# NathanBWaters/playaid_core

Hardware: AMD Instinct MI355X
Metric: 1080p frames/sec end-to-end (higher is better)
Workload: dtype f32; 1 GPU; configs[1]: 64 x 1080x1920 BGR frames per GPU per clip; parallelism=single GPU, lanes=2, ingest=raw BGR frames resident in HBM

## Files before the change

include/playaid_hip.h:

```cpp
#ifndef PLAYAID_HIP_H
#define PLAYAID_HIP_H

#include <stddef.h>
#include <stdint.h>

#ifdef __cplusplus
extern "C" {
#endif

#define PA_ABI_VERSION 15
#define PA_WEIGHT_MAGIC 0x31574150
#define PA_LSTM_MAGIC 0x314c4150
#define PA_ENCODER_MAGIC 0x31454150
#define PA_FEATURE_STRIDE 1024
#define PA_CROP 128

typedef enum pa_status {
    PA_OK = 0,
    PA_ERR_INVALID_ARG = -1,
    PA_ERR_HIP = -2,
    PA_ERR_BAD_WEIGHTS = -3,
    PA_ERR_CAPACITY = -4,
    PA_ERR_NO_DEVICE = -5,
    PA_ERR_NOT_READY = -6,
// ... 316 lines not shown
int pa_wino_conv3x3_splitk(const float* x, const float* ug, const float* bias, const float* residual, float* out, int32_t n,
                           int32_t height, int32_t width, int32_t cin, int32_t cout, int32_t bn, int32_t in_px_stride, int32_t out_px_stride,
                           int32_t out_pad, int32_t act, int32_t res_after, float* slab, size_t slab_floats, int32_t* tickets,
                           int32_t n_tickets, void* stream);

size_t pa_conv_weight_bytes(int32_t cin, int32_t cout, int32_t ksize, int32_t compute_dtype, int32_t has_residual);
int pa_conv_pack_weights(const float* w_host, int32_t cin, int32_t cout, int32_t ksize, int32_t compute_dtype, int32_t has_residual,
                         void* out_host);
int pa_conv2d(const float* x, const void* w, const float* bias, const float* residual, float* out, int32_t n, int32_t height,
              int32_t width, int32_t cin, int32_t cout, int32_t ksize, int32_t stride, int32_t in_pad, int32_t in_px_stride,
              int32_t out_px_stride, int32_t out_pad, int32_t act, int32_t res_after, int32_t compute_dtype, void* stream);
int pa_conv2d_branch(const float* x, const void* w, const float* bias, const float* residual, float* out, const float* w2, float* out2,
                     int32_t n, int32_t height, int32_t width, int32_t cin, int32_t cout, int32_t ksize, int32_t stride, int32_t in_pad,
                     int32_t in_px_stride, int32_t out_px_stride, int32_t out_pad, int32_t act, int32_t res_after, int32_t compute_dtype,
                     void* stream);

typedef struct pa_encoder pa_encoder;
size_t pa_encoder_blob_bytes(int32_t in_dim, int32_t hidden_dim, int32_t slots, int32_t enc_dim, int32_t num_layers,
                             int32_t ff_dim, int32_t num_actions);
int pa_encoder_create(int32_t device, int32_t in_dim, int32_t hidden_dim, int32_t slots, int32_t enc_dim, int32_t num_heads,
                      int32_t num_layers, int32_t ff_dim, int32_t num_actions, int32_t max_rows, const void* blob_host,
                      size_t blob_bytes, pa_encoder** out);
void pa_encoder_destroy(pa_encoder* h);
const char* pa_encoder_last_error(const pa_encoder* h);
int pa_encoder_forward(pa_encoder* h, const float* feats, int32_t ld, int32_t seq_len, int32_t batch, float* logp, void* stream);


int pa_profile_enable(pa_engine* e, int32_t on);
int pa_profile_read(pa_engine* e, pa_kernel_stat* stats, int32_t max_stats, int32_t* n_stats);

// ... 48 lines not shown
```

playaid_core_amd/_lib.py:

```python
from __future__ import annotations

import ctypes as C
import os

HERE = os.path.dirname(os.path.abspath(__file__))
LIB_PATH = os.environ.get("PA_LIB_PATH") or os.path.join(HERE, "libplayaid_hip.so")

PA_ABI_VERSION = 15
PA_DTYPE_F32 = 0
PA_DTYPE_BF16 = 1
PA_DTYPE_EMULATED_F32 = 2
DTYPES = {"f32": PA_DTYPE_F32, "bf16": PA_DTYPE_BF16, "emulated_f32": PA_DTYPE_EMULATED_F32}
PA_WEIGHT_MAGIC = 0x31574150
PA_LSTM_MAGIC = 0x314C4150
PA_ENCODER_MAGIC = 0x31454150
PA_FEATURE_STRIDE = 1024
PA_TRACE_STAGES = 20
DET_FORMS = ("not_run", "stem_direct", "stem_bf16", "wino", "patch", "pgemm", "pgemm_up", "psgemm", "psgemm_up", "igemm", "sppf",
             "maxpool", "upsample", "absorbed", "decode", "bgemm", "bgemm_up")
CN_FORMS = ("not_run", "stem_pool", "avgpool", "wino", "patch", "igemm_128x128", "igemm_128x64", "igemm_64x64", "psgemm",
            "bgemm", "bgemm_splitk", "avgpool_bf16")
LSTM_FORMS = ("not_run", "steps", "u1", "u2", "u4", "u8", "mfma")

PA_OK = 0
# ... 167 lines not shown
    ("pa_convnet_forward", C.c_int, [_P, _P, C.c_int32, _P, C.c_int32, _P]),
    ("pa_convnet_trace", C.c_int, [_P, _P, C.c_int32, C.c_int32, C.c_int32, _P, C.c_size_t, _P]),
    ("pa_convnet_layer_forms", C.c_int, [_P, _P, C.c_int32]),
    ("pa_detector_plan", C.c_int, [_P] * 5 + [C.c_int32] + [_P] * 7),
    ("pa_detector_plan_desc", C.c_int, [_P, _P, _P, C.c_int32, C.c_int32, C.c_longlong, _P, C.c_int32, C.c_longlong, _P]),
    ("pa_square_crops_src", C.c_int, [_P, _P, C.c_int32, C.c_int32, C.c_int32, _P, _P, C.c_int32, C.c_int32, C.c_int32, _P, _P, _P]),
    ("pa_wino_weight_floats", C.c_size_t, [C.c_int32, C.c_int32]),
    ("pa_wino_channels_per_workgroup", C.c_int, [C.c_int32, C.c_int64]),
    ("pa_wino_transform_weights", C.c_int, [_P, C.c_int32, C.c_int32, C.c_int32, _P]),
    ("pa_wino_conv3x3", C.c_int, [_P, _P, _P, _P, _P] + [C.c_int32] * 11 + [_P]),
    ("pa_conv_weight_bytes", C.c_size_t, [C.c_int32] * 5),
    ("pa_conv_pack_weights", C.c_int, [_P] + [C.c_int32] * 5 + [_P]),
    ("pa_conv2d", C.c_int, [_P, _P, _P, _P, _P] + [C.c_int32] * 14 + [_P]),
    ("pa_conv2d_branch", C.c_int, [_P, _P, _P, _P, _P, _P, _P] + [C.c_int32] * 14 + [_P]),
    ("pa_wino_conv3x3_splitk", C.c_int, [_P, _P, _P, _P, _P] + [C.c_int32] * 11 + [_P, C.c_size_t, _P, C.c_int32, _P]),
    ("pa_crop_resize_width", C.c_int, [_P, _P, C.c_int32, C.c_int32, C.c_int32, C.POINTER(C.c_int32), C.c_int32, C.c_int32, _P, C.c_int32,
                                       C.POINTER(C.c_int32), _P]),
    ("pa_encoder_blob_bytes", C.c_size_t, [C.c_int32] * 7),
    ("pa_encoder_create", C.c_int, [C.c_int32] * 10 + [_P, C.c_size_t, C.POINTER(_P)]),
    ("pa_encoder_destroy", None, [_P]),
    ("pa_encoder_last_error", C.c_char_p, [_P]),
    ("pa_encoder_forward", C.c_int, [_P, _P, C.c_int32, C.c_int32, C.c_int32, _P, _P]),
    ("pa_mjpeg_create", C.c_int, [C.c_int32, C.c_int32, C.c_int32, C.c_int32, C.c_size_t, C.POINTER(_P)]),
    ("pa_mjpeg_destroy", None, [_P]),
    ("pa_mjpeg_last_error", C.c_char_p, [_P]),
    ("pa_mjpeg_probe", C.c_int, [_P, C.c_size_t, C.POINTER(C.c_int32), C.c_char_p, C.c_size_t]),
    ("pa_mjpeg_set_sync_rounds", C.c_int, [_P, C.c_int32]),
    ("pa_mjpeg_set_groups", C.c_int, [_P, C.c_int32]),
    ("pa_mjpeg_last_sync_rounds", C.c_int, [_P]),
    ("pa_mjpeg_debug_counters", C.c_int, [_P]),
# ... 55 lines not shown
```

playaid_core_amd/conv.py:

```python
from __future__ import annotations

import ctypes as C

import numpy as np
import torch

from . import _lib


def pack_weights(w_oihw: np.ndarray, compute_dtype: str = "emulated_f32", has_residual: bool = False) -> np.ndarray:
    lib = _lib.load()
    w = np.ascontiguousarray(np.asarray(w_oihw, dtype=np.float32).transpose(0, 2, 3, 1))
    cout, k, _, cin = w.shape
    dt = _lib.DTYPES[compute_dtype]
    nbytes = lib.pa_conv_weight_bytes(cin, cout, k, dt, int(has_residual))
    if nbytes == 0:
        raise ValueError("cin and cout must be multiples of 32, the kernel 1x1 or 3x3, the dtype 'f32' or 'emulated_f32'")
    out = np.empty(nbytes, dtype=np.uint8)
    rc = lib.pa_conv_pack_weights(w.ctypes.data_as(C.c_void_p), cin, cout, k, dt, int(has_residual), out.ctypes.data_as(C.c_void_p))
    if rc:
        raise ValueError(f"pa_conv_pack_weights: status {rc}")
    return out


# ... 27 lines not shown
    n, hp, wp, cs = x_pad.shape
    h, wd = hp - 2 * in_pad, wp - 2 * in_pad
    oh, ow = h // stride, wd // stride
    mk = lambda: torch.zeros((n, oh + 2 * out_pad, ow + 2 * out_pad, cout), dtype=torch.float32, device=x_pad.device)
    out = mk() if out is None else out
    out2 = mk() if out2 is None else out2
    if out2.shape != out.shape:
        raise ValueError("out2 is addressed like out: same shape")
    ptr = lambda t_: C.c_void_p(t_.data_ptr()) if t_ is not None else C.c_void_p(0)
    stream = C.c_void_p(torch.cuda.current_stream(x_pad.device).cuda_stream)
    rc = lib.pa_conv2d_branch(ptr(x_pad), ptr(w), ptr(bias), C.c_void_p(0), ptr(out), ptr(w2), ptr(out2), n, h, wd, cin, cout, ksize, stride, in_pad, cs,
                              out.shape[3], out_pad, int(act), 0, _lib.DTYPES[compute_dtype], stream)
    if rc:
        raise ValueError(f"pa_conv2d_branch: status {rc}")
    return out, out2
```

playaid_core_amd/csrc/conv_rows.hip:

```cpp
#include "conv_rows.h"
#include "../../include/playaid_hip.h"

namespace pa {

GemmParams conv_row_params(const ConvRow& r) {
    const int oh = r.in_h / r.stride, ow = r.in_w / r.stride;
    const int in_hb = r.in_h + 2 * r.in_pad, in_wb = r.in_w + 2 * r.in_pad;
    const int out_hb = oh + 2 * r.out_pad, out_wb = ow + 2 * r.out_pad;
    GemmParams p;
    memset(&p, 0, sizeof(p));
    p.M = r.images * oh * ow;
    p.N = r.cout;
    p.taps = r.ksize * r.ksize;
    p.kw_taps = r.ksize;
    p.chunk = r.cin;
    p.ktot = p.taps * p.chunk;
    p.howo = oh * ow;
    p.wo = ow;
    p.in_px_stride = r.in_px_stride;
    p.in_row_stride = in_wb * r.in_px_stride;
    p.in_img_stride = in_hb * in_wb * r.in_px_stride;
    p.stride = r.stride;
    p.off_y = p.off_x = r.in_pad - (r.ksize - 1) / 2;
    p.out_px_stride = r.out_px_stride;
// ... 145 lines not shown
    const int oh = height / 2, ow = width / 2;
    const int in_wb = width + 2 * in_pad, in_hb = height + 2 * in_pad, out_wb = ow + 2 * out_pad, out_hb = oh + 2 * out_pad;
    if ((long long)n * in_hb * in_wb * in_px_stride >= (1ll << 29) || (long long)n * out_hb * out_wb * out_px_stride >= (1ll << 29)) return PA_ERR_CAPACITY;
    pa::GemmParams p = pa::conv_row_params({ n,  height, width, in_pad, in_px_stride,  cin, cout, 3, 2,
                                             out_pad, out_px_stride,  act, 0});
    p.act = x;
    p.wgt = static_cast<const float*>(w);
    p.bias = bias;
    p.out = out;
    p.wgt2 = w2;
    p.out2 = out2;
    const hipError_t e = pa::launch_pgemm(p, 64, static_cast<hipStream_t>(stream));
    return e == hipSuccess ? PA_OK : (e == hipErrorInvalidValue ? PA_ERR_INVALID_ARG : PA_ERR_HIP);
}

}
```

playaid_core_amd/csrc/igemm.hip:

```cpp
#include "tile_common.h"
#include <cstdio>
#include <cstdlib>

namespace pa {

#ifndef PA_COUNTED_VMCNT
#define PA_COUNTED_VMCNT 0
#endif

template <int BM, int BN, int BK, bool GATHER, int ABL = 0, bool SKIPW = false>
__global__ __launch_bounds__(256) void igemm_f32_kernel(const GemmParams p) {
    constexpr int MI = BM / 64;
    constexpr int NI = BN / 64;
    using Stage = Im2colStage<4, BK, BM, BN, GATHER>;
    constexpr int LDS_STRIDE = BK;
    constexpr int A_ROWS = Stage::A_ROWS, B_ROWS = Stage::B_ROWS;
    constexpr int STAGE = (BM + BN) * LDS_STRIDE;
    __shared__ __attribute__((aligned(16))) float lds[3 * STAGE];

    Stage st;
    st.setup(p);
    const int tile_m = st.tile_m, tile_n = st.tile_n, z = st.z;
    const int ks_begin = st.ks_begin, ks_end = st.ks_end;
    const int tid = threadIdx.x;
    const int wave_id = __builtin_amdgcn_readfirstlane(tid >> 6);
#define PA_ISSUE_STAGE(BUF)                                                \
    {                                                                      \
        float* As_w = lds + (BUF) * STAGE + wave_id * 256;                 \
        st.issue(p, As_w, As_w + BM * LDS_STRIDE);                         \
    }

    const int lane = tid & 63;
    const int wave = tid >> 6;
    const int wm = wave >> 1, wn = wave & 1;
    const int lr = lane & 31;
    const int lh = lane >> 5;
// ... 2 lines not shown
#pragma unroll
    for (int mi = 0; mi < MI; ++mi)
#pragma unroll
        for (int ni = 0; ni < NI; ++ni)
#pragma unroll
            for (int e = 0; e < 16; ++e) acc[mi][ni][e] = 0.f;

    const int a_rd_off = (wm * (BM / 2) + lr) * LDS_STRIDE;
    const int b_rd_off = BM * LDS_STRIDE + (wn * (BN / 2) + lr) * LDS_STRIDE;
    const int swz = BK == 32 ? ((lr >> 1) & 7) : (lr & 15);

    constexpr int TS = BN;
    constexpr int CPR = BN / 4;
    constexpr int ROWS_PP = 256 / CPR;
    constexpr int EP_IT = BM / ROWS_PP;
    static_assert(BM * TS <= 3 * STAGE, "transposed tile must fit the LDS ring");
    const bool direct_out = p.splitk <= 1;
    const int c4 = (tid & (CPR - 1)) * 4;
    const int r_t = tid / CPR;
    int o_t[EP_IT];
    f32x4 res_t[EP_IT];
#pragma unroll
    for (int i = 0; i < EP_IT; ++i) {
        int m = tile_m * BM + r_t + ROWS_PP * i;
        m = m < p.M ? m : p.M - 1;
        int img, oy, ox;
        split_m(p, m, img, oy, ox);
        o_t[i] = img * p.out_img_stride + (oy + p.out_pad) * p.out_row_stride + (ox + p.out_pad) * p.out_px_stride +
                 tile_n * BN + c4;
        res_t[i] = f32x4{0.f, 0.f, 0.f, 0.f};
    }
    if (direct_out && p.residual) {
#pragma unroll
        for (int i = 0; i < EP_IT; ++i) res_t[i] = *reinterpret_cast<const f32x4*>(p.residual + o_t[i]);
    }
    f32x4 bias4 = f32x4{0.f, 0.f, 0.f, 0.f};
    if (direct_out && p.bias) bias4 = *reinterpret_cast<const f32x4*>(p.bias + tile_n * BN + c4);

    f32x4 af[2][MI], bf[2][NI];
#define PA_LOAD_FRAGS(SET, STAGE_PTR, KK)                                                                     \
    {                                                                                                         \
        const int ch = (((KK) * 2 + lh) ^ swz) * 4;                                                           \
        _Pragma("unroll") for (int mi = 0; mi < MI; ++mi)                                                     \
            af[SET][mi] = *reinterpret_cast<const f32x4*>((STAGE_PTR) + a_rd_off + mi * 32 * LDS_STRIDE + ch); \
        _Pragma("unroll") for (int ni = 0; ni < NI; ++ni)                                                     \
            bf[SET][ni] = *reinterpret_cast<const f32x4*>((STAGE_PTR) + b_rd_off + ni * 32 * LDS_STRIDE + ch); \
    }
#ifdef PA_ABLATION_BUILD
    const unsigned long long clk_t0 = __builtin_amdgcn_s_memtime(), clk_r0 = __builtin_amdgcn_s_memrealtime();
#endif
    if (ks_begin < ks_end) PA_ISSUE_STAGE(0);
    if (ks_begin + 1 < ks_end) PA_ISSUE_STAGE(1);
// ... 57 lines not shown
        p.clk[1] = __builtin_amdgcn_s_memrealtime() - clk_r0;
    }
#endif

    float* const tbuf = lds;
#pragma unroll
    for (int mi = 0; mi < MI; ++mi)
#pragma unroll
        for (int ni = 0; ni < NI; ++ni)
#pragma unroll
            for (int e = 0; e < 16; ++e) {
                const int row = wm * (BM / 2) + mi * 32 + (e & 3) + 8 * (e >> 2) + 4 * lh;
                tbuf[row * TS + wn * (BN / 2) + ni * 32 + lr] = acc[mi][ni][e];
            }
    __syncthreads();
#pragma unroll
    for (int i = 0; i < EP_IT; ++i) {
        const int row = r_t + ROWS_PP * i;
        const int m = tile_m * BM + row;
        if (m >= p.M) continue;
        f32x4 v = *reinterpret_cast<const f32x4*>(tbuf + row * TS + c4);
        if (!direct_out) {
            *reinterpret_cast<f32x4*>(p.slab + ((size_t)z * p.M + m) * p.N + tile_n * BN + c4) = v;
        } else {
            *reinterpret_cast<f32x4*>(p.out + o_t[i]) = epilogue4(v, bias4, res_t[i], p.relu, p.res_after);
        }
    }
}

template <typename OutT> __global__ __launch_bounds__(256) void splitk_reduce_kernel(const GemmParams p) {
    constexpr bool BF16 = sizeof(OutT) == 2;
    const OutT* residual = reinterpret_cast<const OutT*>(p.residual);
    OutT* out = reinterpret_cast<OutT*>(p.out);
    const int n4 = p.N >> 2;
    const size_t total = (size_t)p.M * n4;
    for (size_t i = (size_t)blockIdx.x * blockDim.x + threadIdx.x; i < total; i += (size_t)gridDim.x * blockDim.x) {
        const int m = (int)(i / n4);
        const int n = (int)(i - (size_t)m * n4) * 4;
        f32x4 s = *reinterpret_cast<const f32x4*>(p.slab + (size_t)m * p.N + n);
        for (int z = 1; z < p.splitk; ++z) s += *reinterpret_cast<const f32x4*>(p.slab + ((size_t)z * p.M + m) * p.N + n);
// ... 12 lines not shown
            ov.x = f32_to_bf16(s.x); ov.y = f32_to_bf16(s.y); ov.z = f32_to_bf16(s.z); ov.w = f32_to_bf16(s.w);
            *reinterpret_cast<ushort4*>(out + o) = ov;
        } else {
            f32x4 rv = f32x4{0.f, 0.f, 0.f, 0.f};
            if (residual) rv = *reinterpret_cast<const f32x4*>(residual + o);
            if (!p.res_after) s += rv;
            s = act4(s, p.relu);
            if (p.res_after) s += rv;
            *reinterpret_cast<f32x4*>(out + o) = s;
        }
    }
}

template <int BM, int BN, int BK>
static hipError_t launch_tile(const GemmParams& p, hipStream_t s) {
    const int grid = p.tiles_m * p.tiles_n * p.splitk;
#ifdef PA_ABLATION_BUILD
    static const int abl = getenv("PA_ABLATE") ? atoi(getenv("PA_ABLATE")) : 0;
    static unsigned long long* clk_dev = nullptr;
    static int clk_calls = 0;
    if (getenv("PA_CLK") && !p.gather) {
        if (!clk_dev) (void)hipMalloc(&clk_dev, 16);
        GemmParams q = p;
        q.clk = clk_dev;
        hipLaunchKernelGGL((igemm_f32_kernel<BM, BN, BK, false, 0>), dim3(grid), dim3(256), 0, s, q);
        if (++clk_calls % 97 == 0) {
            unsigned long long h[2];
            (void)hipMemcpy(h, clk_dev, 16, hipMemcpyDeviceToHost);
            fprintf(stderr, "[igemm clk] tile %dx%dx%d M=%d N=%d K=%d: %llu cycles / %llu x10ns -> %.3f GHz\n", BM, BN, BK, p.M, p.N, p.ktot, h[0], h[1], (double)h[0] / (double)h[1] * 0.1);
        }
        return hipGetLastError();
// ... 10 lines not shown
    else
        hipLaunchKernelGGL((igemm_f32_kernel<BM, BN, BK, false>), dim3(grid), dim3(256), 0, s, p);
    return hipGetLastError();
}

hipError_t launch_igemm(const GemmParams& p_in, GemmTile tile, hipStream_t s) {
    GemmParams p = p_in;
    TileDims d = tile_dims(tile, 4);
    if (p.chunk % d.bk != 0 || p.k2_steps) {
        tile = tile == TILE_128x64_K64 ? TILE_128x64 : TILE_64x64;
        d = tile_dims(tile, 4);
    }
    const int bm = d.bm, bn = d.bn, bk = d.bk;
    if (p.N % bn != 0 || p.chunk % bk != 0 || p.ktot != p.taps * p.chunk + p.k2_steps * 32 || p.M <= 0) return hipErrorInvalidValue;
    if (p.k2_steps && (bk != 32 || !p.act2 || p.gather)) return hipErrorInvalidValue;
    fill_pow2_shifts(p);
    p.tiles_m = (p.M + bm - 1) / bm;
    p.tiles_n = p.N / bn;
    plan_splitk(p.ktot / bk, p.splitk, p.ksteps_per_split);
    hipError_t err;
    switch (tile) {
        case TILE_128x128: err = launch_tile<128, 128, 32>(p, s); break;
        case TILE_128x64: err = launch_tile<128, 64, 32>(p, s); break;
        case TILE_64x64: err = launch_tile<64, 64, 32>(p, s); break;
        case TILE_128x64_K64: err = launch_tile<128, 64, 64>(p, s); break;
        default: err = launch_tile<64, 64, 64>(p, s); break;
    }
    if (err != hipSuccess) return err;
    if (p.splitk_used) *p.splitk_used = p.splitk;
    if (p.splitk > 1 && !p.defer_reduce) return launch_splitk_reduce(p, s);
    return hipSuccess;
}

hipError_t launch_splitk_reduce(const GemmParams& p, hipStream_t s, bool out_bf16) {
    const size_t total = (size_t)p.M * (p.N >> 2);
    int grid = (int)((total + 255) / 256);
    if (grid > 2048) grid = 2048;
    if (out_bf16) hipLaunchKernelGGL(splitk_reduce_kernel<bf16_t>, dim3(grid), dim3(256), 0, s, p);
    else hipLaunchKernelGGL(splitk_reduce_kernel<float>, dim3(grid), dim3(256), 0, s, p);
    return hipGetLastError();
}

}
```

playaid_core_amd/csrc/pa_api.hip:

```cpp
#include "../../include/playaid_hip.h"
#include "conv_rows.h"

#include <algorithm>
#include <cmath>
#include <cstdio>
#include <cstdlib>
#include <cstring>
#include <string>
#include <vector>

using namespace pa;

namespace {

constexpr int WINO_TICKETS = 4096;

struct ConvLayer {
    std::string name;
    int cin, cout, kh, kw, stride;
    int in_hw, out_hw;
    int in_pad, out_pad;
    int off;
    int taps, kw_taps, chunk;
    int in_px_stride;
    float* in = nullptr;
    float* out = nullptr;
    float* residual = nullptr;
    float* wgt = nullptr;
    float* wino_wgt = nullptr;
    int wino_bn = 0;
// ... 49 lines not shown
    double* clean_g6 = nullptr;
    size_t clean_g6_cap = 0;
    float* x0 = nullptr;
    float* x0_slot[2] = {nullptr, nullptr};
    int32_t* pre_status[2] = {nullptr, nullptr};
    float* pooled = nullptr;
    float* feats_tmp = nullptr;
    float* cache = nullptr;
    int32_t* cache_status = nullptr;
    float* h1 = nullptr;
    int32_t* gather = nullptr;
    int gather_key[4] = {-1, -1, -1, -1};
    float* slab = nullptr;
    size_t slab_floats = 0;
    float* wino_tickets = nullptr;
    std::vector<ConvLayer> convs;
    ConvLayer fc;
    float* stem_wgt_bf16 = nullptr;
    float* c1 = nullptr;
    float* p1 = nullptr;
    float* layer4_out = nullptr;
    float* w1d = nullptr;
    float* b1d = nullptr;
    float *w2 = nullptr, *b2 = nullptr, *w3 = nullptr, *b3 = nullptr;
    GemmTile head_tile = TILE_64x64;
    int head_splitk = 16;
    CropPlan* plans = nullptr;
    int32_t* coef = nullptr;
    int coef_dim = 0;
    int32_t* coef_cache = nullptr;
// ... 276 lines not shown
        p.act2 = at(L.in2, (size_t)crop0 * w2 * w2 * L.in2_c);
        p.k2_steps = L.in2_c / (bf ? 64 : 32);
        p.in2_px_stride = L.in2_c;
        p.in2_row_stride = w2 * L.in2_c;
        p.in2_img_stride = w2 * w2 * L.in2_c;
        p.stride2 = L.in2_stride;
        p.off2 = 1;
        p.ktot += L.in2_c;
    }
    GemmTile tile = L.tile;
    int splitk = L.splitk;
    if (!L.forced) choose_tile(p.M, p.N, p.ktot / (bf ? 64 : 32), &tile, &splitk);
    p.splitk = splitk;
    const size_t slab_avail = e->slab_floats > slab_off ? e->slab_floats - slab_off : 0;
    if ((size_t)p.splitk * p.M * p.N > slab_avail) p.splitk = 1;
    const bool f32_branch = !bf && !e->emu && L.ds_next_wgt;
    const bool f32_branch_here = f32_branch && p.splitk <= 1;
    const bool ds_here = (bf && L.ds_next_wgt) || f32_branch_here;
    if (bf && L.ds_next_wgt) {
        p.wgt2 = L.ds_next_wgt;
        p.out2 = at(L.ds_next_out, crop0 * out_crop);
    }
    if ((bf && L.ds_next_wgt) || (bf && L.ds_probe)) {
        tile = (p.N % 128 == 0 && ((p.M + 127) / 128) * (p.N / 128) >= 256) ? TILE_128x128 : TILE_128x64;
        p.splitk = 1;
    }
    const double k_main = ((bf_ds || f32_ds) ? L.k_alg - L.in2_c : L.k_alg) + (ds_here ? L.cin : 0);
    const double flops = 2.0 * p.M * p.N * k_main;
    const double bytes = (double)es * ((double)ncrops * L.in_hw * L.in_hw * L.cin + (double)p.M * p.N * ((L.residual || bf_ds || f32_ds || ds_here) ? 2 : 1) +
                                       (double)p.N * k_main + ((L.in2 && !bf_ds && !f32_ds) ? (double)ncrops * L.in2_hw * L.in2_hw * L.in2_c : 0.0));
    const bool as_wino = !bf && L.wino_wgt && !p.act2;
    bool branch_left = f32_branch;
    {
        ProfScope ps(e, s, prof_name, flops, bytes, as_wino ? flops * 4.0 / 9.0 : flops);
        static const int use_patch = getenv("PA_PATCH") ? atoi(getenv("PA_PATCH")) : 1;
        static const int use_bf16_patch = getenv("PA_BF16_PATCH") ? atoi(getenv("PA_BF16_PATCH")) : 1;
        if (e->emu && L.split_wgt && !p.act2 && !p.residual) {
            HIPCHK(e, launch_psgemm(p, L.split_wgt, (size_t)ncrops * out_crop, 0, s));
        } else if (bf) {
            hipError_t pe = hipErrorInvalidValue;
            if (use_bf16_patch && L.stride == 1 && !p.act2) pe = launch_conv3x3_bf16_patch(p, s);
            if (pe == hipErrorInvalidValue) {
                static const int t256 = getenv("PA_BF16_T256") ? atoi(getenv("PA_BF16_T256")) : 1;
                if (t256 && !p.out2 && tile == TILE_128x128 && p.splitk == 1 && ((p.M + 255) / 256) * (p.N / 128) >= 256) tile = TILE_256x128;
                pe = launch_igemm_bf16(p, tile, s);
            }
            HIPCHK(e, pe);
// ... 15 lines not shown
            if (pe == hipErrorInvalidValue) pe = launch_igemm(p, tile, s);
            HIPCHK(e, pe);
        } else {
            static const int use_pgemm = getenv("PA_S2_PGEMM") ? atoi(getenv("PA_S2_PGEMM")) : 2;
            hipError_t pe = hipErrorInvalidValue;
            const bool pg = use_pgemm && L.kh == 3 && L.stride == 2 && !p.act2 && !p.residual && p.splitk <= 1 && !p.gather;
            if (pg && f32_branch_here) {
                p.wgt2 = L.ds_next_wgt;
                p.out2 = at(L.ds_next_out, crop0 * out_crop);
                pe = launch_pgemm(p, 64, s);
                if (pe == hipSuccess) branch_left = false;
                p.wgt2 = nullptr;
                p.out2 = nullptr;
            }
            if (pg && pe == hipErrorInvalidValue) pe = launch_pgemm(p, use_pgemm == 2 ? 64 : 0, s);
            if (pe == hipErrorInvalidValue) pe = launch_igemm(p, tile, s);
            HIPCHK(e, pe);
        }
    }
    if (branch_left) {
        const GemmParams d = branch_gemm_of(L.in, L.in_hw, L.cin, L.stride, L.ds_next_wgt, L.ds_next_out);
        ProfScope ps(e, s, e->profile_layers ? L.ds_next_name.c_str() : prof_name, 2.0 * d.M * d.N * L.cin,
                     4.0 * ((double)ncrops * L.in_hw * L.in_hw * L.cin / (L.stride * L.stride) + (double)d.M * d.N + (double)d.N * L.cin));
        HIPCHK(e, launch_f32_branch(d));
    }
    return PA_OK;
}

int run_backbone_part(pa_engine* e, int crop0, int ncrops, const float* x_in, float* feats_out, size_t slab_off, hipStream_t s,
                      int stop = PA_TRACE_STAGES) {
    int rc;
    ConvLayer stem = e->convs[0];
    stem.in = const_cast<float*>(x_in);
// ... 445 lines not shown
                    static const int wino_ds = getenv("PA_WINO_DS") ? atoi(getenv("PA_WINO_DS")) : 1;
                    static const int wino_min_hw = getenv("PA_WINO_MIN_HW") ? atoi(getenv("PA_WINO_MIN_HW")) : 4;
                    if (wino_mode && wino_ds && hw_out >= wino_min_hw && hw_out % 4 == 0) {
                        L.wino_bn = wino_pick_bn(co, (long long)NC * (hw_out / 4) * (hw_out / 4), co);
                        std::vector<float> ug(wino_weight_floats(co, co), 0.f);
                        if (!br.dry) wino_transform_weights(keep_w.data(), co, co, L.wino_bn, ug.data());
                        rc = upload(e, &L.wino_wgt, ug);
                        if (rc) return rc;
                        rc = upload(e, &L.ds_wgt, wd);
                        if (rc) return rc;
                        if (e->emu && (rc = upload_split(e, &L.ds_split_wgt, wd, co, cin, false))) return rc;
                        ALLOC(L.ds_out, buf, true);
                        static const int f32_ds_fuse = getenv("PA_F32_DS_FUSE") ? atoi(getenv("PA_F32_DS_FUSE")) : 1;
                        static const int ds_side_knob = getenv("PA_DS_SIDE") ? atoi(getenv("PA_DS_SIDE")) : 0;
                        static const int s2_pgemm_knob = getenv("PA_S2_PGEMM") ? atoi(getenv("PA_S2_PGEMM")) : 2;
                        ConvLayer& C1 = e->convs[e->convs.size() - 2];
                        if (f32_ds_fuse && !ds_side_knob && s2_pgemm_knob && !e->emu && li < 3 && C1.in == cur && C1.kh == 3 &&
                            C1.stride == 2 && C1.cout == co && C1.out_hw == hw_out && C1.out_pad == L.out_pad && C1.chunk == cin && C1.cin == cin &&
                            C1.in_hw == hw_in[li] && C1.in_pad == 1 && !C1.forced) {
                            C1.ds_next_wgt = L.ds_wgt;
                            C1.ds_next_out = L.ds_out;
                            C1.ds_next_name = L.name;
                            L.ds_fused = true;
                        }
                    }
                }
                rc = upload(e, &L.bias, bf);
                if (rc) return rc;
                L.in2 = cur;
                L.in2_c = cin;
                L.in2_hw = hw_in[li];
                L.in2_stride = stride;
// ... 73 lines not shown
        HIPCHK(e, hipMemcpy(e->arena, e->arena_stage.data(), e->arena_used, hipMemcpyHostToDevice));
        std::vector<uint8_t>().swap(e->arena_stage);
    }
    {
        size_t need = 0;
        for (const ConvLayer& L : e->convs)
            if (L.splitk > 1) need = std::max(need, (size_t)L.splitk * NC * L.out_hw * L.out_hw * L.cout);
        if (e->fc.splitk > 1) need = std::max(need, (size_t)e->fc.splitk * NC * PA_FEATURE_STRIDE);
        if (e->head_splitk > 1) need = std::max(need, (size_t)e->head_splitk * NC * 512);
        bool any_wino = false;
        for (const ConvLayer& L : e->convs) any_wino = any_wino || L.wino_wgt;
        if (any_wino) {
            need = std::max(need, (size_t)256 * 512 * 32);
            ALLOC(e->wino_tickets, (size_t)2 * WINO_TICKETS, true);
        }
        need *= 2;
        e->slab_floats = need;
        ALLOC(e->slab, need, false);
    }
    e->coef_dim = std::max(cfg->max_frame_height, cfg->max_frame_width);
    e->t_stride = std::max((size_t)cfg->max_frame_height * cfg->max_frame_width * 3, (size_t)(448 + 128) * PA_CROP * 3);
    ALLOC(e->plans, (size_t)NC, true);
    ALLOC(e->fallback, (size_t)NC + 4, true);
    ALLOC(e->coef, (size_t)NC * 2 * e->coef_dim * (2 + PA_KSIZE_MAX), false);
    e->coef_cache_dmax = std::min(std::min(cfg->max_frame_height, cfg->max_frame_width), 1024);
    ALLOC(e->coef_cache, coef_cache_ints(e->coef_cache_dmax), false);
    e->coef_cache_pad = 30;
    HIPCHK(e, launch_build_coef_cache(e->coef_cache, e->coef_cache_pad, e->coef_cache_dmax, nullptr));
    ALLOC(e->area_tabs, (size_t)NC * 2 * PA_CROP, true);
    ALLOC(e->t1, (size_t)NC * e->t_stride, false);
// ... 903 lines not shown
```

playaid_core_amd/csrc/tile_common.h:

```cpp
#pragma once
#include "pa_kernels.h"

namespace pa {


typedef float f32x16 __attribute__((ext_vector_type(16)));
typedef float f32x4 __attribute__((ext_vector_type(4)));
typedef float f32x2 __attribute__((ext_vector_type(2)));
typedef uint32_t u32x4 __attribute__((ext_vector_type(4)));
typedef __bf16 bf16x8 __attribute__((ext_vector_type(8)));
typedef uint16_t bf16_t;

__device__ __forceinline__ int xcd_remap(int b, int nwg) {
    const int q = nwg >> 3, r = nwg & 7, xcd = b & 7;
    return (xcd < r ? xcd * (q + 1) : r * (q + 1) + (xcd - r) * q) + (b >> 3);
}

__device__ __forceinline__ void xcd_grid_tile(int xcd, int rank, int gm, int gn, int tiles_m, int tiles_n, int& tile_m, int& tile_n) {
    const int tm_per = tiles_m / gm, tn_per = tiles_n / gn;
    const int xm = xcd / gn, lm = rank / tn_per;
    tile_m = xm * tm_per + lm;
    tile_n = (xcd - xm * gn) * tn_per + (rank - lm * tn_per);
}

// ... 55 lines not shown
struct Im2colStage {
    static constexpr int CH = BK * EB / 16;
    static constexpr int PASS_ROWS = 256 / CH;
    static constexpr int A_ROWS = BM / PASS_ROWS;
    static constexpr int B_ROWS = BN / PASS_ROWS;
    static constexpr int CE = 16 / EB;

    int z, tile_m, tile_n;
    int row0, colq;
    int a_off[A_ROWS], a_off2[A_ROWS], b_off[B_ROWS];
    int nk_main, ks_begin, ks_end;
    int issue_ks;
    int cur_kc, cur_kx, cur_ky;
    __amdgpu_buffer_rsrc_t act_rs, wgt_rs, act2_rs;

    __device__ __forceinline__ void setup(const GemmParams& p) {
        const int wg = xcd_remap(blockIdx.x, gridDim.x);
        const int tiles_mn = p.tiles_m * p.tiles_n;
        z = wg / tiles_mn;
        const int t_id = wg - z * tiles_mn;
        tile_m = t_id / p.tiles_n;
        tile_n = t_id - tile_m * p.tiles_n;

        const int tid = threadIdx.x;
        row0 = tid / CH;
        colq = (tid & (CH - 1)) ^ (CH == 8 ? ((row0 >> 1) & 7) : (row0 & 15));
#pragma unroll
        for (int i = 0; i < A_ROWS; ++i) {
            int m = tile_m * BM + row0 + PASS_ROWS * i;
            m = m < p.M ? m : p.M - 1;
            a_off2[i] = 0;
            if (GATHER) {
// ... 124 lines not shown
```

Measured before the change: 64330 frames/s.

## Fuse split-K reduction and downsample branch into the im2col GEMM kernel

When split-K is used, each workgroup writes its partial tile to the slab and takes an atomic ticket. The last arriver sums all partials and applies bias, residual and activation, so the separate split-K reduce kernel launch goes away. Extra grid blocks also compute the stride-2 1x1 downsample branch GEMM inside the same launch instead of as a separate kernel. This allows the f32 downsample fusion for more layers, but adds ticket atomics, global-memory round trips through the slab, and tail serialization on last arrivers.

```diff
diff --git a/include/playaid_hip.h b/include/playaid_hip.h
--- a/include/playaid_hip.h
+++ b/include/playaid_hip.h
@@ -354,6 +354,10 @@
                      int32_t n, int32_t height, int32_t width, int32_t cin, int32_t cout, int32_t ksize, int32_t stride, int32_t in_pad,
                      int32_t in_px_stride, int32_t out_px_stride, int32_t out_pad, int32_t act, int32_t res_after, int32_t compute_dtype,
                      void* stream);
+int pa_igemm_conv2d(const float* x, const float* w, const float* bias, const float* residual, float* out, const float* w2, float* out2,
+                    int32_t n, int32_t height, int32_t width, int32_t cin, int32_t cout, int32_t ksize, int32_t stride, int32_t in_pad,
+                    int32_t in_px_stride, int32_t out_px_stride, int32_t out_pad, int32_t act, int32_t res_after, int32_t splitk,
+                    int32_t fused, float* slab, size_t slab_floats, int32_t* tickets, int32_t n_tickets, void* stream);
 
 typedef struct pa_encoder pa_encoder;
 size_t pa_encoder_blob_bytes(int32_t in_dim, int32_t hidden_dim, int32_t slots, int32_t enc_dim, int32_t num_layers,
diff --git a/playaid_core_amd/_lib.py b/playaid_core_amd/_lib.py
--- a/playaid_core_amd/_lib.py
+++ b/playaid_core_amd/_lib.py
@@ -205,6 +205,7 @@
     ("pa_conv2d", C.c_int, [_P, _P, _P, _P, _P] + [C.c_int32] * 14 + [_P]),
     ("pa_conv2d_branch", C.c_int, [_P, _P, _P, _P, _P, _P, _P] + [C.c_int32] * 14 + [_P]),
     ("pa_wino_conv3x3_splitk", C.c_int, [_P, _P, _P, _P, _P] + [C.c_int32] * 11 + [_P, C.c_size_t, _P, C.c_int32, _P]),
+    ("pa_igemm_conv2d", C.c_int, [_P] * 7 + [C.c_int32] * 15 + [_P, C.c_size_t, _P, C.c_int32, _P]),
     ("pa_crop_resize_width", C.c_int, [_P, _P, C.c_int32, C.c_int32, C.c_int32, C.POINTER(C.c_int32), C.c_int32, C.c_int32, _P, C.c_int32,
                                        C.POINTER(C.c_int32), _P]),
     ("pa_encoder_blob_bytes", C.c_size_t, [C.c_int32] * 7),
diff --git a/playaid_core_amd/conv.py b/playaid_core_amd/conv.py
--- a/playaid_core_amd/conv.py
+++ b/playaid_core_amd/conv.py
@@ -65,3 +65,38 @@
     if rc:
         raise ValueError(f"pa_conv2d_branch: status {rc}")
     return out, out2
+
+
+class IgemmScratch:
+
+    def __init__(self, device="cuda:0", slab_floats: int = 1 << 22, n_tickets: int = 4096):
+        self.slab = torch.empty(slab_floats, dtype=torch.float32, device=device)
+        self.tickets = torch.zeros(n_tickets, dtype=torch.int32, device=device)
+
+
+def igemm_conv2d(x_pad: torch.Tensor, w: torch.Tensor, cin: int, cout: int, ksize: int, stride: int = 1, splitk: int = 1, fused: bool = True,
+                 scratch: IgemmScratch = None, in_pad: int = None, bias=None, residual=None, out=None, w2=None, out2=None, out_pad: int = 0,
+                 act: int = 0, res_after: bool = False):
+    lib = _lib.load()
+    if x_pad.dtype != torch.float32 or not x_pad.is_cuda or not x_pad.is_contiguous() or x_pad.dim() != 4:
+        raise ValueError("x_pad: contiguous float32[n, H + 2 pad, W + 2 pad, C] on the device")
+    in_pad = (ksize - 1) // 2 if in_pad is None else in_pad
+    n, hp, wp, cs = x_pad.shape
+    h, wd = hp - 2 * in_pad, wp - 2 * in_pad
+    oh, ow = h // stride, wd // stride
+    mk = lambda: torch.zeros((n, oh + 2 * out_pad, ow + 2 * out_pad, cout), dtype=torch.float32, device=x_pad.device)
+    out = mk() if out is None else out
+    if w2 is not None:
+        out2 = mk() if out2 is None else out2
+        if out2.shape != out.shape:
+            raise ValueError("out2 is addressed like out: same shape")
+    ptr = lambda t_: C.c_void_p(t_.data_ptr()) if t_ is not None else C.c_void_p(0)
+    slab = scratch.slab if scratch is not None else None
+    tickets = scratch.tickets if scratch is not None else None
+    stream = C.c_void_p(torch.cuda.current_stream(x_pad.device).cuda_stream)
+    rc = lib.pa_igemm_conv2d(ptr(x_pad), ptr(w), ptr(bias), ptr(residual), ptr(out), ptr(w2), ptr(out2), n, h, wd, cin, cout, ksize, stride, in_pad, cs,
+                             out.shape[3], out_pad, int(act), int(bool(res_after)), int(splitk), int(bool(fused)),
+                             ptr(slab), slab.numel() if slab is not None else 0, ptr(tickets), tickets.numel() if tickets is not None else 0, stream)
+    if rc:
+        raise ValueError(f"pa_igemm_conv2d: status {rc}")
+    return (out, out2) if w2 is not None else out
diff --git a/playaid_core_amd/csrc/conv_rows.hip b/playaid_core_amd/csrc/conv_rows.hip
--- a/playaid_core_amd/csrc/conv_rows.hip
+++ b/playaid_core_amd/csrc/conv_rows.hip
@@ -1,4 +1,5 @@
 #include "conv_rows.h"
+#include "tile_common.h"
 #include "../../include/playaid_hip.h"
 
 namespace pa {
@@ -183,4 +184,56 @@
     return e == hipSuccess ? PA_OK : (e == hipErrorInvalidValue ? PA_ERR_INVALID_ARG : PA_ERR_HIP);
 }
 
-}
+int pa_igemm_conv2d(const float* x, const float* w, const float* bias, const float* residual, float* out, const float* w2, float* out2, int32_t n,
+                    int32_t height, int32_t width, int32_t cin, int32_t cout, int32_t ksize, int32_t stride, int32_t in_pad, int32_t in_px_stride,
+                    int32_t out_px_stride, int32_t out_pad, int32_t act, int32_t res_after, int32_t splitk, int32_t fused, float* slab,
+                    size_t slab_floats, int32_t* tickets, int32_t n_tickets, void* stream) {
+    if (!x || !w || !out || n <= 0 || height <= 0 || width <= 0 || (ksize != 1 && ksize != 3) || (stride != 1 && stride != 2) || height % stride || width % stride ||
+        in_pad < (ksize - 1) / 2 || in_px_stride < cin || out_px_stride < cout || out_pad < 0 || act < 0 || act > 2 || splitk < 1 || cin <= 0 || cin % 32 ||
+        cout <= 0 || cout % 64)
+        return PA_ERR_INVALID_ARG;
+    if ((w2 != nullptr) != (out2 != nullptr) || (w2 && (ksize != 3 || stride != 2 || in_px_stride != cin))) return PA_ERR_INVALID_ARG;
+    auto misaligned = [](const void* q) { return (reinterpret_cast<unsigned long long>(q) & 15ull) != 0; };
+    if (in_px_stride % 4 || out_px_stride % 4 || misaligned(x) || misaligned(w) || misaligned(out) || misaligned(residual) || misaligned(w2) || misaligned(out2) ||
+        misaligned(bias))
+        return PA_ERR_INVALID_ARG;
+    const int oh = height / stride, ow = width / stride;
+    const int in_wb = width + 2 * in_pad, in_hb = height + 2 * in_pad, out_wb = ow + 2 * out_pad, out_hb = oh + 2 * out_pad;
+    if ((long long)n * in_hb * in_wb * in_px_stride >= (1ll << 29) || (long long)n * out_hb * out_wb * out_px_stride >= (1ll << 29)) return PA_ERR_CAPACITY;
+    pa::GemmParams p = pa::conv_row_params({ n,  height, width, in_pad, in_px_stride,  cin, cout, ksize, stride,
+                                             out_pad, out_px_stride,  act, res_after ? 1 : 0});
+    const pa::GemmTile tile = pa::im2col_tile(p.M, p.N);
+    const pa::TileDims d = pa::tile_dims(tile, 4);
+    const long long tiles = (long long)((p.M + d.bm - 1) / d.bm) * (p.N / d.bn);
+    if (splitk > 1) {
+        if (!slab || misaligned(slab) || slab_floats < (size_t)splitk * p.M * p.N || (size_t)splitk * p.M * p.N >= ((size_t)1 << 29)) return PA_ERR_INVALID_ARG;
+        if (fused && (!tickets || n_tickets < tiles)) return PA_ERR_INVALID_ARG;
+    }
+    p.act = x;
+    p.wgt = w;
+    p.bias = bias;
+    p.residual = residual;
+    p.out = out;
+    p.slab = slab;
+    p.splitk = splitk;
+    hipStream_t s = static_cast<hipStream_t>(stream);
+    hipError_t e;
+    if (fused) {
+        p.tickets = tickets;
+        p.wgt2 = w2;
+        p.out2 = out2;
+        e = pa::launch_igemm(p, tile, s);
+    } else {
+        e = pa::launch_igemm(p, tile, s);
+        if (e == hipSuccess && w2) {
+            pa::GemmParams b = pa::conv_row_params({n, height, width, in_pad, in_px_stride, cin, cout, 1, 2, out_pad, out_px_stride, 0, 0});
+            b.act = x;
+            b.wgt = w2;
+            b.out = out2;
+            e = pa::launch_igemm(b, tile, s);
+        }
+    }
+    return e == hipSuccess ? PA_OK : (e == hipErrorInvalidValue ? PA_ERR_INVALID_ARG : PA_ERR_HIP);
+}
+
+}
diff --git a/playaid_core_amd/csrc/igemm.hip b/playaid_core_amd/csrc/igemm.hip
--- a/playaid_core_amd/csrc/igemm.hip
+++ b/playaid_core_amd/csrc/igemm.hip
@@ -19,7 +19,24 @@
     __shared__ __attribute__((aligned(16))) float lds[3 * STAGE];
 
     Stage st;
-    st.setup(p);
+    bool second = false;
+    if constexpr (GATHER) {
+        st.setup(p);
+    } else {
+        const int tiles_mn = p.tiles_m * p.tiles_n, main_grid = tiles_mn * p.splitk, b = blockIdx.x;
+        second = b >= main_grid;
+        st.setup(p, second ? main_grid + xcd_remap(b - main_grid, tiles_mn) : xcd_remap(b, main_grid));
+        if (second) {
+#pragma unroll
+            for (int i = 0; i < B_ROWS; ++i)
+                st.b_off[i] = (st.tile_n * BN + st.row0 + Stage::PASS_ROWS * i - 4) * p.chunk + st.colq * Stage::CE;
+            st.wgt_rs = glds_rsrc(p.wgt2);
+            st.ks_begin = st.issue_ks = 0;
+            st.ks_end = st.nk_main = p.chunk / BK;
+            st.cur_kc = 0;
+            st.cur_ky = st.cur_kx = 1;
+        }
+    }
     const int tile_m = st.tile_m, tile_n = st.tile_n, z = st.z;
     const int ks_begin = st.ks_begin, ks_end = st.ks_end;
     const int tid = threadIdx.x;
@@ -52,8 +69,12 @@
     constexpr int CPR = BN / 4;
     constexpr int ROWS_PP = 256 / CPR;
     constexpr int EP_IT = BM / ROWS_PP;
-    static_assert(BM * TS <= 3 * STAGE, "transposed tile must fit the LDS ring");
-    const bool direct_out = p.splitk <= 1;
+    static_assert(BM * TS < 3 * STAGE, "transposed tile (and the last-arriver word behind it) must fit the LDS ring");
+    const bool direct_out = p.splitk <= 1 || second;
+    const float* const bias_p = second ? nullptr : p.bias;
+    const float* const res_p = second ? nullptr : p.residual;
+    float* const out_p = second ? p.out2 : p.out;
+    const int relu = second ? 0 : p.relu;
     const int c4 = (tid & (CPR - 1)) * 4;
     const int r_t = tid / CPR;
     int o_t[EP_IT];
@@ -68,12 +89,12 @@
                  tile_n * BN + c4;
         res_t[i] = f32x4{0.f, 0.f, 0.f, 0.f};
     }
-    if (direct_out && p.residual) {
-#pragma unroll
-        for (int i = 0; i < EP_IT; ++i) res_t[i] = *reinterpret_cast<const f32x4*>(p.residual + o_t[i]);
+    if (direct_out && res_p) {
+#pragma unroll
+        for (int i = 0; i < EP_IT; ++i) res_t[i] = *reinterpret_cast<const f32x4*>(res_p + o_t[i]);
     }
     f32x4 bias4 = f32x4{0.f, 0.f, 0.f, 0.f};
-    if (direct_out && p.bias) bias4 = *reinterpret_cast<const f32x4*>(p.bias + tile_n * BN + c4);
+    if (direct_out && bias_p) bias4 = *reinterpret_cast<const f32x4*>(bias_p + tile_n * BN + c4);
 
     f32x4 af[2][MI], bf[2][NI];
 #define PA_LOAD_FRAGS(SET, STAGE_PTR, KK)                                                                     \
@@ -161,6 +182,49 @@
                 tbuf[row * TS + wn * (BN / 2) + ni * 32 + lr] = acc[mi][ni][e];
             }
     __syncthreads();
+    if constexpr (!GATHER) {
+        if (!direct_out && p.tickets) {
+            constexpr int SC = 17;
+            const int mn_bytes = p.M * p.N * 4;
+            const __amdgpu_buffer_rsrc_t slab_rs = glds_rsrc(p.slab, p.splitk * mn_bytes);
+            int s_off[EP_IT];
+#pragma unroll
+            for (int i = 0; i < EP_IT; ++i) {
+                const int row = r_t + ROWS_PP * i;
+                const int m = tile_m * BM + row;
+                s_off[i] = (m * p.N + tile_n * BN + c4) * 4;
+                if (m >= p.M) continue;
+                const f32x4 v = *reinterpret_cast<const f32x4*>(tbuf + row * TS + c4);
+                __builtin_amdgcn_raw_buffer_store_b128((u32x4)v, slab_rs, s_off[i], z * mn_bytes, SC);
+            }
+            asm volatile("s_waitcnt vmcnt(0)" ::: "memory");
+            float* const last_w = lds + 3 * STAGE - 1;
+            __syncthreads();
+            if (tid == 0) {
+                int32_t* const tk = p.tickets + tile_m * p.tiles_n + tile_n;
+                const int drawn = __hip_atomic_fetch_add(tk, 1, __ATOMIC_RELAXED, __HIP_MEMORY_SCOPE_AGENT);
+                if (drawn == p.splitk - 1) __hip_atomic_store(tk, 0, __ATOMIC_RELAXED, __HIP_MEMORY_SCOPE_AGENT);
+                *last_w = drawn == p.splitk - 1 ? 1.f : 0.f;
+            }
+            __syncthreads();
+            if (*last_w == 0.f) return;
+            if (p.bias) bias4 = *reinterpret_cast<const f32x4*>(p.bias + tile_n * BN + c4);
+#pragma unroll
+            for (int i = 0; i < EP_IT; ++i) {
+                if (tile_m * BM + r_t + ROWS_PP * i >= p.M) continue;
+                f32x4 s = (f32x4)__builtin_amdgcn_raw_buffer_load_b128(slab_rs, s_off[i], 0, SC);
+                for (int zz = 1; zz < p.splitk; ++zz) s += (f32x4)__builtin_amdgcn_raw_buffer_load_b128(slab_rs, s_off[i], zz * mn_bytes, SC);
+                if (p.bias) s += bias4;
+                f32x4 rv = f32x4{0.f, 0.f, 0.f, 0.f};
+                if (p.residual) rv = *reinterpret_cast<const f32x4*>(p.residual + o_t[i]);
+                if (!p.res_after) s += rv;
+                s = act4(s, p.relu);
+                if (p.res_after) s += rv;
+                *reinterpret_cast<f32x4*>(p.out + o_t[i]) = s;
+            }
+            return;
+        }
+    }
 #pragma unroll
     for (int i = 0; i < EP_IT; ++i) {
         const int row = r_t + ROWS_PP * i;
@@ -170,7 +234,7 @@
         if (!direct_out) {
             *reinterpret_cast<f32x4*>(p.slab + ((size_t)z * p.M + m) * p.N + tile_n * BN + c4) = v;
         } else {
-            *reinterpret_cast<f32x4*>(p.out + o_t[i]) = epilogue4(v, bias4, res_t[i], p.relu, p.res_after);
+            *reinterpret_cast<f32x4*>(out_p + o_t[i]) = epilogue4(v, bias4, res_t[i], relu, p.res_after);
         }
     }
 }
@@ -213,7 +277,7 @@
 
 template <int BM, int BN, int BK>
 static hipError_t launch_tile(const GemmParams& p, hipStream_t s) {
-    const int grid = p.tiles_m * p.tiles_n * p.splitk;
+    const int grid = p.tiles_m * p.tiles_n * (p.splitk + (p.out2 ? 1 : 0));
 #ifdef PA_ABLATION_BUILD
     static const int abl = getenv("PA_ABLATE") ? atoi(getenv("PA_ABLATE")) : 0;
     static unsigned long long* clk_dev = nullptr;
@@ -254,10 +318,17 @@
     const int bm = d.bm, bn = d.bn, bk = d.bk;
     if (p.N % bn != 0 || p.chunk % bk != 0 || p.ktot != p.taps * p.chunk + p.k2_steps * 32 || p.M <= 0) return hipErrorInvalidValue;
     if (p.k2_steps && (bk != 32 || !p.act2 || p.gather)) return hipErrorInvalidValue;
+    if ((p.wgt2 != nullptr) != (p.out2 != nullptr)) return hipErrorInvalidValue;
+    if (p.out2 && (p.taps != 9 || p.kw_taps != 3 || p.stride != 2 || p.in_px_stride != p.chunk || p.gather || p.k2_steps || p.defer_reduce || p.skip_w))
+        return hipErrorInvalidValue;
+#ifdef PA_ABLATION_BUILD
+    if (p.out2) return hipErrorInvalidValue;
+#endif
     fill_pow2_shifts(p);
     p.tiles_m = (p.M + bm - 1) / bm;
     p.tiles_n = p.N / bn;
     plan_splitk(p.ktot / bk, p.splitk, p.ksteps_per_split);
+    if (p.splitk <= 1 || p.defer_reduce || p.gather || !p.slab || (size_t)p.splitk * p.M * p.N >= ((size_t)1 << 29)) p.tickets = nullptr;
     hipError_t err;
     switch (tile) {
         case TILE_128x128: err = launch_tile<128, 128, 32>(p, s); break;
@@ -268,7 +339,7 @@
     }
     if (err != hipSuccess) return err;
     if (p.splitk_used) *p.splitk_used = p.splitk;
-    if (p.splitk > 1 && !p.defer_reduce) return launch_splitk_reduce(p, s);
+    if (p.splitk > 1 && !p.defer_reduce && !p.tickets) return launch_splitk_reduce(p, s);
     return hipSuccess;
 }
 
diff --git a/playaid_core_amd/csrc/pa_api.hip b/playaid_core_amd/csrc/pa_api.hip
--- a/playaid_core_amd/csrc/pa_api.hip
+++ b/playaid_core_amd/csrc/pa_api.hip
@@ -14,6 +14,7 @@
 namespace {
 
 constexpr int WINO_TICKETS = 4096;
+constexpr int IGEMM_TICKETS = 4096;
 
 struct ConvLayer {
     std::string name;
@@ -93,6 +94,7 @@
     float* slab = nullptr;
     size_t slab_floats = 0;
     float* wino_tickets = nullptr;
+    int32_t* igemm_tickets = nullptr;
     std::vector<ConvLayer> convs;
     ConvLayer fc;
     float* stem_wgt_bf16 = nullptr;
@@ -399,8 +401,12 @@
     p.splitk = splitk;
     const size_t slab_avail = e->slab_floats > slab_off ? e->slab_floats - slab_off : 0;
     if ((size_t)p.splitk * p.M * p.N > slab_avail) p.splitk = 1;
+    static const int igemm_fuse = getenv("PA_IGEMM_FUSE") ? atoi(getenv("PA_IGEMM_FUSE")) : 1;
+    if (igemm_fuse && !bf && !e->emu && p.splitk > 1 && e->igemm_tickets && (size_t)((p.M + 63) / 64) * (p.N / 64) <= (size_t)IGEMM_TICKETS)
+        p.tickets = e->igemm_tickets + (slab_off ? IGEMM_TICKETS : 0);
     const bool f32_branch = !bf && !e->emu && L.ds_next_wgt;
     const bool f32_branch_here = f32_branch && p.splitk <= 1;
+    const bool f32_branch_grouped = f32_branch && p.splitk > 1 && p.tickets;
     const bool ds_here = (bf && L.ds_next_wgt) || f32_branch_here;
     if (bf && L.ds_next_wgt) {
         p.wgt2 = L.ds_next_wgt;
@@ -416,6 +422,7 @@
                                        (double)p.N * k_main + ((L.in2 && !bf_ds && !f32_ds) ? (double)ncrops * L.in2_hw * L.in2_hw * L.in2_c : 0.0));
     const bool as_wino = !bf && L.wino_wgt && !p.act2;
     bool branch_left = f32_branch;
+    bool branch_grouped = false;
     {
         ProfScope ps(e, s, prof_name, flops, bytes, as_wino ? flops * 4.0 / 9.0 : flops);
         static const int use_patch = getenv("PA_PATCH") ? atoi(getenv("PA_PATCH")) : 1;
@@ -461,9 +468,22 @@
                 p.out2 = nullptr;
             }
             if (pg && pe == hipErrorInvalidValue) pe = launch_pgemm(p, use_pgemm == 2 ? 64 : 0, s);
+            if (pe == hipErrorInvalidValue && f32_branch_grouped) {
+                p.wgt2 = L.ds_next_wgt;
+                p.out2 = at(L.ds_next_out, crop0 * out_crop);
+                pe = launch_igemm(p, tile, s);
+                if (pe == hipSuccess) branch_left = false, branch_grouped = true;
+                p.wgt2 = nullptr;
+                p.out2 = nullptr;
+            }
             if (pe == hipErrorInvalidValue) pe = launch_igemm(p, tile, s);
             HIPCHK(e, pe);
         }
+    }
+    if (branch_grouped) {
+        const GemmParams d = branch_gemm_of(L.in, L.in_hw, L.cin, L.stride, L.ds_next_wgt, L.ds_next_out);
+        ProfScope ps(e, s, e->profile_layers ? L.ds_next_name.c_str() : prof_name, 2.0 * d.M * d.N * L.cin,
+                     4.0 * ((double)ncrops * L.in_hw * L.in_hw * L.cin / (L.stride * L.stride) + (double)d.M * d.N + (double)d.N * L.cin));
     }
     if (branch_left) {
         const GemmParams d = branch_gemm_of(L.in, L.in_hw, L.cin, L.stride, L.ds_next_wgt, L.ds_next_out);
@@ -939,8 +959,9 @@
                         static const int f32_ds_fuse = getenv("PA_F32_DS_FUSE") ? atoi(getenv("PA_F32_DS_FUSE")) : 1;
                         static const int ds_side_knob = getenv("PA_DS_SIDE") ? atoi(getenv("PA_DS_SIDE")) : 0;
                         static const int s2_pgemm_knob = getenv("PA_S2_PGEMM") ? atoi(getenv("PA_S2_PGEMM")) : 2;
+                        static const int igemm_fuse_knob = getenv("PA_IGEMM_FUSE") ? atoi(getenv("PA_IGEMM_FUSE")) : 1;
                         ConvLayer& C1 = e->convs[e->convs.size() - 2];
-                        if (f32_ds_fuse && !ds_side_knob && s2_pgemm_knob && !e->emu && li < 3 && C1.in == cur && C1.kh == 3 &&
+                        if (f32_ds_fuse && !ds_side_knob && s2_pgemm_knob && !e->emu && (li < 3 || igemm_fuse_knob) && C1.in == cur && C1.kh == 3 &&
                             C1.stride == 2 && C1.cout == co && C1.out_hw == hw_out && C1.out_pad == L.out_pad && C1.chunk == cin && C1.cin == cin &&
                             C1.in_hw == hw_in[li] && C1.in_pad == 1 && !C1.forced) {
                             C1.ds_next_wgt = L.ds_wgt;
@@ -1044,6 +1065,7 @@
             need = std::max(need, (size_t)256 * 512 * 32);
             ALLOC(e->wino_tickets, (size_t)2 * WINO_TICKETS, true);
         }
+        ALLOC(e->igemm_tickets, (size_t)2 * IGEMM_TICKETS, true);
         need *= 2;
         e->slab_floats = need;
         ALLOC(e->slab, need, false);
diff --git a/playaid_core_amd/csrc/tile_common.h b/playaid_core_amd/csrc/tile_common.h
--- a/playaid_core_amd/csrc/tile_common.h
+++ b/playaid_core_amd/csrc/tile_common.h
@@ -93,8 +93,8 @@
     int cur_kc, cur_kx, cur_ky;
     __amdgpu_buffer_rsrc_t act_rs, wgt_rs, act2_rs;
 
-    __device__ __forceinline__ void setup(const GemmParams& p) {
-        const int wg = xcd_remap(blockIdx.x, gridDim.x);
+    __device__ __forceinline__ void setup(const GemmParams& p) { setup(p, xcd_remap(blockIdx.x, gridDim.x)); }
+    __device__ __forceinline__ void setup(const GemmParams& p, int wg) {
         const int tiles_mn = p.tiles_m * p.tiles_n;
         z = wg / tiles_mn;
         const int t_id = wg - z * tiles_mn;
```

Result: no change. 64680 frames/s (median of 6 runs) (+0.5%).
